# rookiepig/CrossScalePatchMatch

Hardware: AMD Instinct MI355X
Metric: Mpix/s disparity (GRD, use_cs=true) (higher is better)
Workload: dtype f64; 1 GPU; C3: 1242x375 max_dis=128 GRD scale_num=5 reg_lambda=0.3 wnd=35 iters=3 (BASELINE.json configs[2] when C3); cc_name=GRD, schedule=raster, sweep_cells=as cost_source, raster_sweep=persistent, rb_rounds=1, sweep_workgroups_per_cu=2, sweep_workgroup_waves=levels - 1 (coarsest level folded, CSPM_OPT_SWEEP_FOLD), early_exit=True, pairs_per_gpu=22, distinct_pairs_per_gpu=22, pairs_in_flight_per_gpu=2, use_pp=False, parallelism=1 rank(s), one per GPU, 2 independent pair stream(s) each, dispatch=every rank generates its own pairs (no collective in the timed region)

## Files before the change

### crossscalepatchmatch_amd/csrc/cspm_chain.h

```cpp
#pragma once
#include <type_traits>
#include "cspm_tap.h"

#pragma clang fp contract(off)

namespace cspm {

struct ChainScratch {
  double part[2][kMaxPasses * kWave];
};
struct ChainPlane { double a, b, c; };

struct ChainLevel {
  int W, H, n, Dm1;
  int ox0, oy0;
  int r_lo, nrows;
  int passes, nsteps;
  int Wp, pad;
  bool has_valid;
  double maxc;
  const char *px, *opx;
  const char *gx, *ogx;
  int dirE;
  double sgn;
  const double *vol;
  const char *vol2;
  size_t slab;
  uint32_t Ip;
};

template <int SRC>
__device__ __forceinline__ ChainLevel make_chain_level(const Cost &cd, int s, int view, int cx, int cy) {
  const Level &L = cd.lv[s];
  constexpr int E = elem_size<SRC>();
  ChainLevel A;
  A.W = L.W; A.H = L.H; A.n = cd.n; A.Dm1 = L.D - 1;
  A.ox0 = cx - cd.half; A.oy0 = cy - cd.half;
  A.r_lo = max(0, -A.oy0);
  const int r_hi = min(cd.n - 1, L.H - 1 - A.oy0);
  A.nrows = r_hi - A.r_lo + 1;
  A.passes = (A.nrows + kChainRows - 1) / kChainRows;
  A.nsteps = (cd.n + kRowMod - 1) / kRowMod;
  A.Wp = L.Wp; A.pad = L.pad;
  A.has_valid = L.D >= 2;
  A.maxc = cd.max_cost[view * CSPM_MAX_LEVELS + s];
  A.vol2 = nullptr;
  A.gx = A.ogx = nullptr;
  if (SRC == kSrcCenGrd) { A.gx = reinterpret_cast<const char *>(L.grd[view]); A.ogx = reinterpret_cast<const char *>(L.grd[1 - view]); }
  if (SRC == kSrcVol2) {
    A.px = reinterpret_cast<const char *>(L.pix[view]); A.opx = A.px;
    A.Ip = L.pix[view][cy * L.Wp + L.pad + cx];
    A.vol2 = reinterpret_cast<const char *>(L.vol2[view]);
    A.Dm1 = max(L.D - 1, 1);
  } else if (census_elem<SRC>()) {
    A.px = reinterpret_cast<const char *>(L.pc[view]); A.opx = reinterpret_cast<const char *>(L.pc[1 - view]);
    A.Ip = L.pc[view][cy * L.Wp + L.pad + cx].pix;
  } else if (SRC == kSrcGrd8) {
    A.px = reinterpret_cast<const char *>(L.px8[view]); A.opx = reinterpret_cast<const char *>(L.px8[1 - view]);
    A.Ip = pix8_colour(L.px8[view][cy * L.Wp + L.pad + cx].hi);
  } else {
    A.px = reinterpret_cast<const char *>(L.px[view]); A.opx = reinterpret_cast<const char *>(L.px[1 - view]);
    A.Ip = L.px[view][cy * L.Wp + L.pad + cx].pix;
  }
  A.Ip = (uint32_t)__builtin_amdgcn_readfirstlane((int)A.Ip);
  A.sgn = view == 0 ? -1.0 : 1.0;
  A.dirE = view == 0 ? -E : E;
  A.vol = L.vol[view];
  A.slab = (size_t)L.W * (size_t)L.H;
  return A;
}

#ifdef CSPM_SWEEP_TRACE
constexpr int kTraceSlots = 16;
__shared__ long long *s_tr;
#define EVAL_STAMP(slot) do { if (wave == 0 && lane == 0 && s_tr) s_tr[slot] = wall_clock64(); } while (0)
#else
#define EVAL_STAMP(slot) do { } while (0)
#endif

__device__ __forceinline__ double wave_uniform(double v) {
  return __hiloint2double(__builtin_amdgcn_readfirstlane(__double2hiint(v)), __builtin_amdgcn_readfirstlane(__double2loint(v)));
}

__device__ __forceinline__ void grd8_cell_pair(const double *lut_a, uint32_t Iq, double XP, const uint4 &pr, bool left, double &c0, double &c1) {
  const double clo = grd8_cell(lut_a, Iq, XP, pix8_colour(pr.y), pix8_x(pr.x, pr.y));
  const double chi = grd8_cell(lut_a, Iq, XP, pix8_colour(pr.w), pix8_x(pr.z, pr.w));
  c0 = left ? chi : clo;
  c1 = left ? clo : chi;
}

template <int SRC, bool ALLV>
__device__ __forceinline__ double chain_tap_value(const Cost &cd, const ChainLevel &A, const Luts &lut, const uint4 &P, double XP, double Pg,
                                                  int of, int qx, int qy, bool ok, double q_disp) {
  constexpr int E = SRC == kSrcVol2 ? 4 : elem_size<SRC>();
  if constexpr (SRC == kSrcImg) {
    const ImgSplit g = split_img(q_disp, A.sgn * q_disp, (double)qx, A.Dm1, A.has_valid);
    const int fxc = min(max(g.fx, -A.pad), A.W + A.pad - 2);
    const int oo = (qy * A.Wp + A.pad + fxc) * E;
    const uint4 o0 = ld_elem<SRC>(A.opx, oo), o1 = ld_elem<SRC>(A.opx, oo + E);
    const double cell = img_cell(pix_of<SRC>(P), g_of(P), pix_of<SRC>(o0), g_of(o0), pix_of<SRC>(o1), g_of(o1), g.fw);
    return g.valid ? cell : A.maxc;
  } else {
    const DispSplit d = ALLV ? split_disp_valid(q_disp) : split_disp(q_disp, A.Dm1, A.has_valid);
    double c0, c1;
    if constexpr (SRC == kSrcVol2) {
      const int cx = ok ? qx : A.ox0 + cd.half;
      const unsigned idx = __umul24((unsigned)d.f, (unsigned)A.slab) + (unsigned)(qy * A.W + cx);
      const double2 cc = *reinterpret_cast<const double2 *>(A.vol2 + (size_t)(idx << 4));
      c0 = cc.x;
      c1 = cc.y;
    } else if constexpr (SRC == kSrcVolume) {
      const int cx = ok ? qx : A.ox0 + cd.half;
      const double *v = A.vol + (size_t)d.f * A.slab + (size_t)qy * A.W + cx;
      c0 = v[0];
      c1 = v[A.slab];
    } else if constexpr (SRC == kSrcGrd8) {
      const bool left = A.dirE < 0;
      const uint4 pr = ld_pix8_pair(A.opx, of + __mul24(A.dirE, d.f) + (left ? -E : 0));
      grd8_cell_pair(lut.a, P.z, XP, pr, left, c0, c1);
    } else if constexpr (SRC == kSrcCenGrd) {
      const int oo = of + __mul24(A.dirE, d.f);
      const uint4 o0 = ld_elem<SRC>(A.opx, oo), o1 = ld_elem<SRC>(A.opx, oo + A.dirE);
      const double g0 = ld_grad(A.ogx, oo >> 1), g1 = ld_grad(A.ogx, (oo + A.dirE) >> 1);
      c0 = cengrd_cell(lut.a, P, Pg, o0, g0);
      c1 = cengrd_cell(lut.a, P, Pg, o1, g1);
    } else {
      const int oo = of + __mul24(A.dirE, d.f);
      cell_pair_of<SRC>(lut.a, P, ld_elem<SRC>(A.opx, oo), ld_elem<SRC>(A.opx, oo + A.dirE), c0, c1);
    }
    return ALLV ? lerp_cells(d.fr, c0, c1) : tap_value(d, c0, c1, A.maxc);
  }
}

template <int SRC, int NC, bool PIPE = false>
__device__ __forceinline__ void chain_passes(const Cost &cd, const ChainLevel &A, const Luts &lut, const ChainPlane (&pl)[NC], int lane,
                                             int pass_first, int pass_step, double *const (&part)[NC]) {
  constexpr int E = SRC == kSrcVol2 ? 4 : elem_size<SRC>();
  const int lutzero = kLutZero;
  const int lr = lane / kRowMod, j = lane - lr * kRowMod;
  if constexpr (PIPE && (SRC == kSrcGrd || SRC == kSrcCen || SRC == kSrcGrd8)) {
    struct PassCtx {
      bool chain_ok;
      int ob;
      double ty[NC];
    };
    struct Fetched {
      uint4 P;
      uint4 o0[NC], o1[NC];
      DispSplit d[NC];
      bool ok;
    };
    const double jd = (double)j;
    const int qx0 = A.ox0 + j;
    auto make_ctx = [&](int p) {
      PassCtx c;
      const int r = p * kChainRows + lr;
      c.chain_ok = (lr < kChainRows) & (r < A.nrows);
      const int row = A.oy0 + A.r_lo + (c.chain_ok ? r : 0);
      c.ob = (row * A.Wp + A.pad + qx0) * E;
#pragma unroll
      for (int k = 0; k < NC; ++k) c.ty[k] = pl[k].b * (double)row + pl[k].c;
      return c;
    };
    auto fetch = [&](const PassCtx &c, int st, Fetched &F) {
      const double xg = (double)(A.ox0 + kRowMod * st);
      const int dx = j + kRowMod * st;
      F.ok = c.chain_ok & (dx < A.n) & ((unsigned)(qx0 + kRowMod * st) < (unsigned)A.W);
      if constexpr (SRC == kSrcGrd8) {
        const uint2 e = ld_pix8(A.px, c.ob + st * (kRowMod * E));
        F.P = uint4{e.x, e.y, 0u, 0u};
      } else {
        F.P = ld_elem<SRC>(A.px, c.ob + st * (kRowMod * E));
      }
#pragma unroll
      for (int k = 0; k < NC; ++k) {
        const double q_disp = tap_disp(pl[k].a, jd, group_disp(pl[k].a, xg, c.ty[k]));
        F.d[k] = split_disp(q_disp, A.Dm1, A.has_valid);
        if constexpr (SRC == kSrcGrd8) {
          F.o0[k] = ld_pix8_pair(A.opx, c.ob + st * (kRowMod * E) + __mul24(A.dirE, F.d[k].f) + (A.dirE < 0 ? -E : 0));
        } else {
          const int of = c.ob + st * (kRowMod * E) + __mul24(A.dirE, F.d[k].f);
          F.o0[k] = ld_elem<SRC>(A.opx, of);
          F.o1[k] = ld_elem<SRC>(A.opx, of + A.dirE);
        }
      }
    };
    auto consume = [&](const Fetched &F, double (&acc)[NC]) {
      uint32_t Iq;
      double XP = 0.0;
      if constexpr (SRC == kSrcGrd8) { Iq = pix8_colour(F.P.y); XP = pix8_x(F.P.x, F.P.y); }
      else Iq = pix_of<SRC>(F.P);
      const int sad0 = (int)__builtin_amdgcn_sad_u8(A.Ip, Iq, 0u);
      const int sad = F.ok ? sad0 : lutzero;
      const double wgt = lut.w[sad];
#pragma unroll
      for (int k = 0; k < NC; ++k) {
        double c0, c1;
        if constexpr (SRC == kSrcGrd8) grd8_cell_pair(lut.a, Iq, XP, F.o0[k], A.dirE < 0, c0, c1);
        else cell_pair_of<SRC>(lut.a, F.P, F.o0[k], F.o1[k], c0, c1);
        acc[k] = __builtin_fma(wgt, tap_value(F.d[k], c0, c1, A.maxc), acc[k]);
      }
    };
    auto copy_fetched = [&](Fetched &d, const Fetched &f) {
      d.P = f.P;
      d.ok = f.ok;
#pragma unroll
      for (int k = 0; k < NC; ++k) { d.o0[k] = f.o0[k]; d.o1[k] = f.o1[k]; d.d[k].valid = f.d[k].valid; d.d[k].f = f.d[k].f; d.d[k].fr = f.d[k].fr; }
    };
    auto copy_ctx = [&](PassCtx &d, const PassCtx &c) {
      d.chain_ok = c.chain_ok;
      d.ob = c.ob;
#pragma unroll
      for (int k = 0; k < NC; ++k) d.ty[k] = c.ty[k];
    };
    if (pass_first >= A.passes) return;
    PassCtx cur = make_ctx(pass_first);
    Fetched F0, F1;
    fetch(cur, 0, F0);
    const int nsteps = A.nsteps;
    for (int p = pass_first; p < A.passes; p += pass_step) {
      const bool has_next = p + pass_step < A.passes;
      PassCtx nxt;
      if (has_next) nxt = make_ctx(p + pass_step);
      else copy_ctx(nxt, cur);
      double acc[NC];
#pragma unroll
      for (int k = 0; k < NC; ++k) acc[k] = 0.0;
      int st = 0;
      for (; st + 1 < nsteps; st += 2) {
        fetch(cur, st + 1, F1);
        __builtin_amdgcn_sched_barrier(0);
        consume(F0, acc);
        const bool in2 = st + 2 < nsteps;
        PassCtx cb;
        cb.chain_ok = in2 ? cur.chain_ok : nxt.chain_ok;
        cb.ob = in2 ? cur.ob : nxt.ob;
#pragma unroll
        for (int k = 0; k < NC; ++k) cb.ty[k] = in2 ? cur.ty[k] : nxt.ty[k];
        fetch(cb, in2 ? st + 2 : 0, F0);
        __builtin_amdgcn_sched_barrier(0);
        consume(F1, acc);
      }
      if (st < nsteps) {
        fetch(nxt, 0, F1);
        __builtin_amdgcn_sched_barrier(0);
        consume(F0, acc);
        copy_fetched(F0, F1);
      }
#pragma unroll
      for (int k = 0; k < NC; ++k) part[k][p * kWave + lane] = acc[k];
      copy_ctx(cur, nxt);
    }
    return;
  }
  bool allv = (SRC == kSrcGrd || census_elem<SRC>() || SRC == kSrcGrd8 || SRC == kSrcVolume || SRC == kSrcVol2) && A.has_valid;
  if (allv) {
    const double x0 = (double)A.ox0, x1 = (double)(A.ox0 + kRowMod * A.nsteps - 1);
    const double y0 = (double)(A.oy0 + A.r_lo), y1 = (double)(A.oy0 + A.r_lo + A.nrows - 1);
    const double lo = 1.0 + 0x1p-20, hi = (double)(A.Dm1 + 1) - 0x1p-20;
#pragma unroll
    for (int c = 0; c < NC; ++c) {
      const double t0 = pl[c].b * y0 + pl[c].c, t1 = pl[c].b * y1 + pl[c].c;
      const double q00 = __builtin_fma(pl[c].a, x0, t0), q01 = __builtin_fma(pl[c].a, x1, t0);
      const double q10 = __builtin_fma(pl[c].a, x0, t1), q11 = __builtin_fma(pl[c].a, x1, t1);
      const double qmin = __builtin_fmin(__builtin_fmin(q00, q01), __builtin_fmin(q10, q11));
      const double qmax = __builtin_fmax(__builtin_fmax(q00, q01), __builtin_fmax(q10, q11));
      allv = allv & (qmin >= lo) & (qmax <= hi);
    }
    allv = __builtin_amdgcn_ballot_w64(!allv) == 0ull;
  }
  auto run_passes = [&](auto allv_tag) {
  constexpr bool ALLV = decltype(allv_tag)::value;
  for (int p = pass_first; p < A.passes; p += pass_step) {
    double acc[NC];
#pragma unroll
    for (int c = 0; c < NC; ++c) acc[c] = 0.0;
    const int r = p * kChainRows + lr;
    const bool chain_ok = (lr < kChainRows) & (r < A.nrows);
    const int dy = A.r_lo + (chain_ok ? r : 0);
    const int qx0 = A.ox0 + j;
    const int ob = ((A.oy0 + dy) * A.Wp + A.pad + qx0) * E;
    double ty[NC];
#pragma unroll
    for (int c = 0; c < NC; ++c) ty[c] = pl[c].b * (double)(A.oy0 + dy) + pl[c].c;
    const double jd = (double)j;
    for (int st = 0; st < A.nsteps; ++st) {
      const double xg = (double)(A.ox0 + kRowMod * st);
      const int dx = j + kRowMod * st;
      const bool ok = chain_ok & (dx < A.n) & ((unsigned)(qx0 + kRowMod * st) < (unsigned)A.W);
      uint4 P;
      double XP = 0.0;
      if constexpr (SRC == kSrcVol2) P = uint4{0u, 0u, *reinterpret_cast<const uint32_t *>(A.px + (size_t)(unsigned)(ob + st * (kRowMod * E))), 0u};
      else if constexpr (SRC == kSrcGrd8) {
        const uint2 e = ld_pix8(A.px, ob + st * (kRowMod * E));
        P = uint4{0u, 0u, pix8_colour(e.y), 0u};
        XP = pix8_x(e.x, e.y);
      } else P = ld_elem<SRC>(A.px, ob + st * (kRowMod * E));
      [[maybe_unused]] double Pg = 0.0;
      if constexpr (SRC == kSrcCenGrd) Pg = ld_grad(A.gx, (ob + st * (kRowMod * E)) >> 1);
      const int sad0 = (int)__builtin_amdgcn_sad_u8(A.Ip, (SRC == kSrcVol2 || SRC == kSrcGrd8) ? P.z : pix_of<SRC>(P), 0u);
      const int sad = ok ? sad0 : lutzero;
      const double wgt = lut.w[sad];
#pragma unroll
      for (int c = 0; c < NC; ++c) {
        const double q_disp = tap_disp(pl[c].a, jd, group_disp(pl[c].a, xg, ty[c]));
        acc[c] = __builtin_fma(wgt, chain_tap_value<SRC, ALLV>(cd, A, lut, P, XP, Pg, ob + st * (kRowMod * E), qx0 + kRowMod * st, A.oy0 + dy, ok, q_disp),
                                acc[c]);
      }
    }
#pragma unroll
    for (int c = 0; c < NC; ++c) part[c][p * kWave + lane] = acc[c];
  }
  };
  if (allv) run_passes(std::true_type{});
  else run_passes(std::false_type{});
}

__device__ __forceinline__ double finish_level(const ChainLevel &A, const double *part, int lane) {
  const int r = lane - A.r_lo;
  const bool in = (r >= 0) & (r < A.nrows);
  const int rc = in ? r : 0;
  const int p = rc / kChainRows, lr = rc - p * kChainRows;
  const double *q = part + p * kWave + lr * kRowMod;
  double R = q[0];
#pragma unroll
  for (int k = 1; k < kRowMod; ++k) R = R + q[k];
  R = in ? R : 0.0;
  return wave_tree_sum(R);
}

template <bool CS, int SRC>
__device__ __forceinline__ double eval_plane_chain(const Cost &cd, const Luts &lut, ChainScratch &m, int view, int x, int y, double nx,
                                                   double ny, double nz, double pa, double pb, double pc, double thresh,
                                                   bool use_thresh, int lane) {
  double cost = 0.0;
  double cur_disp = pa * (double)x + pb * (double)y + pc;
  int cur_x = x, cur_y = y;
  const int levels = CS ? cd.levels : 1;
  for (int s = 0; s < levels; ++s) {
    double a = pa, b = pb, c = pc;
    if (CS) plane_param(nx, ny, nz, (double)cur_x, (double)cur_y, cur_disp, a, b, c);
    const ChainLevel A = make_chain_level<SRC>(cd, s, view, cur_x, cur_y);
    const ChainPlane pl[1] = {{wave_uniform(a), wave_uniform(b), wave_uniform(c)}};
    double *const parts[1] = {m.part[0]};
    wave_lds_fence();
    chain_passes<SRC, 1, true>(cd, A, lut, pl, lane, 0, 1, parts);
    wave_lds_fence();
    const double sc = finish_level(A, m.part[0], lane);
    if (CS) cost += sc * cd.lv[s].wgt;
    else cost = sc;
    if (use_thresh && cost >= thresh) return __builtin_inf();
    cur_y /= 2;
    cur_x /= 2;
    cur_disp /= 2.0;
  }
  return cost;
}

template <bool CS, int SRC>
__global__ __launch_bounds__(kEvalBlock) void k_cost_batch(Cost cd, int view, int n, const int *__restrict__ xy,
                                                           const double *__restrict__ np, double *__restrict__ out) {
  __shared__ LutMem s_lut;
  __shared__ ChainScratch s_m[kEvalBlock / kWave];
  const Luts lut = load_luts(cd, s_lut);
  const int wave = __builtin_amdgcn_readfirstlane((int)(threadIdx.x >> 6));
  const long long e = xcd_block() * (kEvalBlock / kWave) + wave;
  if (e >= n) return;
  const int lane = threadIdx.x & 63;
  const int x = xy[2 * e], y = xy[2 * e + 1];
  const double *p = np + 6 * e;
  const double c = eval_plane_chain<CS, SRC>(cd, lut, s_m[wave], view, x, y, p[0], p[1], p[2], p[3], p[4], p[5], kDoubleMax, false, lane);
  if (lane == 0) out[e] = c;
}

template <bool CS, int SRC>
__global__ __launch_bounds__(kEvalBlock) void k_spatial_rb(Cost cd, Pm pm, int colour, int inc, int nb) {
  __shared__ LutMem s_lut;
  __shared__ ChainScratch s_m[kEvalBlock / kWave];
  const Luts lut = load_luts(cd, s_lut);
  const int halfW = (pm.W + 1) / 2;
  const long long per_view = (long long)halfW * pm.H;
  const int wave = __builtin_amdgcn_readfirstlane((int)(threadIdx.x >> 6));
  const long long e = xcd_block() * (kEvalBlock / kWave) + wave;
  if (e >= 2 * per_view) return;
  const int lane = threadIdx.x & 63;
  const int v = (int)(e / per_view);
  const long long r = e - (long long)v * per_view;
  const int y = (int)(r / halfW);
  const int x = 2 * (int)(r - (long long)y * halfW) + ((y + colour) & 1);
  if (x >= pm.W) return;
  const Field &f = pm.f[v];
  const long long i = (long long)y * pm.W + x;
  Cand best{};
  double best_cost = f.cost[i];
  bool changed = false;
  const bool use_thresh = pm.use_thresh != 0 && *cd.early_ok != 0;
  const int nxs[4] = {x - inc, x, x + inc, x}, nys[4] = {y, y - inc, y, y + inc};
  for (int k = 0; k < nb; ++k) {
    if (nxs[k] < 0 || nxs[k] >= pm.W || nys[k] < 0 || nys[k] >= pm.H) continue;
    const long long j = (long long)nys[k] * pm.W + nxs[k];
    const Cand cand{f.nx[j], f.ny[j], f.nz[j], f.a[j], f.b[j], f.c[j]};
    const double cost = eval_plane_chain<CS, SRC>(cd, lut, s_m[wave], v, x, y, cand.nx, cand.ny, cand.nz, cand.a, cand.b, cand.c, best_cost,
                                                    use_thresh, lane);
    if (cost < best_cost) { best_cost = cost; best = cand; changed = true; }
  }
  if (changed && lane == 0) store_plane(f, i, best.nx, best.ny, best.nz, best.a, best.b, best.c, best_cost);
}

constexpr int kSweepMinWaves = 4;
constexpr int kSweepPollSleep = 1;
constexpr int kSweepPrio = 3;
constexpr int kSweepMaxWaves = CSPM_MAX_LEVELS > kMaxPasses ? CSPM_MAX_LEVELS : kMaxPasses;

struct SweepShared {
  LutMem &lut;
  double (*lvl)[CSPM_MAX_LEVELS];
  ChainScratch *m;
};
__host__ __device__ inline size_t sweep_shared_bytes(int waves) {
  return sizeof(LutMem) + 2 * CSPM_MAX_LEVELS * sizeof(double) + (size_t)(waves < 1 ? 1 : waves) * sizeof(ChainScratch);
}
__device__ __forceinline__ SweepShared sweep_shared(unsigned char *smem) {
  return SweepShared{*reinterpret_cast<LutMem *>(smem), reinterpret_cast<double (*)[CSPM_MAX_LEVELS]>(smem + sizeof(LutMem)),
                     reinterpret_cast<ChainScratch *>(smem + sizeof(LutMem) + 2 * CSPM_MAX_LEVELS * sizeof(double))};
}

template <bool CS, int SRC>
__device__ __forceinline__ ChainLevel sweep_level_setup(const Cost &cd, int v, int x, int y, int wave) {
  if (CS) {
    int cur_x = x, cur_y = y;
    for (int s = 0; s < wave; ++s) { cur_y /= 2; cur_x /= 2; }
    return make_chain_level<SRC>(cd, wave < cd.levels ? wave : 0, v, cur_x, cur_y);
  }
  return make_chain_level<SRC>(cd, 0, v, x, y);
}

template <bool CS, int SRC>
__device__ __forceinline__ void eval_pixel_pair(const Cost &cd, const Luts &lut, const SweepShared &sh, int v, int x, int y, const Cand &c0,
                                                const Cand &c1, bool both, int wave, int lane, double &cost0, double &cost1, const ChainLevel &A) {
  if (CS) {
    const int level = wave;
    double d0 = c0.a * (double)x + c0.b * (double)y + c0.c, d1 = c1.a * (double)x + c1.b * (double)y + c1.c;
    int cur_x = x, cur_y = y;
    for (int s = 0; s < level; ++s) { cur_y /= 2; cur_x /= 2; d0 /= 2.0; d1 /= 2.0; }
    double *part0 = sh.m[level].part[0], *part1 = sh.m[level].part[1];
    if (level < cd.levels) {
      const double wgt = cd.lv[level].wgt;
      ChainPlane pl[2];
      plane_param(c0.nx, c0.ny, c0.nz, (double)cur_x, (double)cur_y, d0, pl[0].a, pl[0].b, pl[0].c);
      pl[0].a = wave_uniform(pl[0].a); pl[0].b = wave_uniform(pl[0].b); pl[0].c = wave_uniform(pl[0].c);
      if (both) {
        plane_param(c1.nx, c1.ny, c1.nz, (double)cur_x, (double)cur_y, d1, pl[1].a, pl[1].b, pl[1].c);
        pl[1].a = wave_uniform(pl[1].a); pl[1].b = wave_uniform(pl[1].b); pl[1].c = wave_uniform(pl[1].c);
        EVAL_STAMP(4);
        double *const parts[2] = {part0, part1};
        chain_passes<SRC, 2>(cd, A, lut, pl, lane, 0, 1, parts);
        EVAL_STAMP(5);
        wave_lds_fence();
        const double s0 = finish_level(A, part0, lane) * wgt;
        const double s1 = finish_level(A, part1, lane) * wgt;
        if (lane == 0) { sh.lvl[0][level] = s0; sh.lvl[1][level] = s1; }
      } else {
        const ChainPlane p1[1] = {pl[0]};
        double *const parts[1] = {part0};
        chain_passes<SRC, 1>(cd, A, lut, p1, lane, 0, 1, parts);
        wave_lds_fence();
        const double s0 = finish_level(A, part0, lane) * wgt;
        if (lane == 0) { sh.lvl[0][level] = s0; sh.lvl[1][level] = s0; }
      }
    }
    const int nw = (int)(blockDim.x >> 6);
    if (cd.levels == nw + 1) {
      const int last = cd.levels - 1;
      double *fold0 = sh.m[nw].part[0], *fold1 = sh.m[nw].part[1];
      ChainLevel B = A;
      if (wave >= 1) {
        double e0 = c0.a * (double)x + c0.b * (double)y + c0.c, e1 = c1.a * (double)x + c1.b * (double)y + c1.c;
        int lx = x, ly = y;
        for (int s = 0; s < last; ++s) { ly /= 2; lx /= 2; e0 /= 2.0; e1 /= 2.0; }
        B = make_chain_level<SRC>(cd, last, v, lx, ly);
        ChainPlane pl[2];
        plane_param(c0.nx, c0.ny, c0.nz, (double)lx, (double)ly, e0, pl[0].a, pl[0].b, pl[0].c);
        pl[0].a = wave_uniform(pl[0].a); pl[0].b = wave_uniform(pl[0].b); pl[0].c = wave_uniform(pl[0].c);
        if (both) {
          plane_param(c1.nx, c1.ny, c1.nz, (double)lx, (double)ly, e1, pl[1].a, pl[1].b, pl[1].c);
          pl[1].a = wave_uniform(pl[1].a); pl[1].b = wave_uniform(pl[1].b); pl[1].c = wave_uniform(pl[1].c);
          double *const parts[2] = {fold0, fold1};
          chain_passes<SRC, 2>(cd, B, lut, pl, lane, wave - 1, nw - 1, parts);
        } else {
          const ChainPlane p1[1] = {pl[0]};
          double *const parts[1] = {fold0};
          chain_passes<SRC, 1>(cd, B, lut, p1, lane, wave - 1, nw - 1, parts);
        }
      }
      __syncthreads();
      if (wave == 1) {
        const double s0 = finish_level(B, fold0, lane) * cd.lv[last].wgt;
        if (lane == 0) { sh.lvl[0][last] = s0; if (!both) sh.lvl[1][last] = s0; }
      } else if (wave == 2 && both) {
        const double s1 = finish_level(B, fold1, lane) * cd.lv[last].wgt;
        if (lane == 0) sh.lvl[1][last] = s1;
      }
    }
    __syncthreads();
    cost0 = cost1 = 0.0;
    if (wave == 0) {
      for (int s = 0; s < cd.levels; ++s) {
        cost0 += sh.lvl[0][s];
        cost1 += sh.lvl[1][s];
      }
    }
  } else {
    const int nw = (int)(blockDim.x >> 6);
    const ChainPlane pl[2] = {{wave_uniform(c0.a), wave_uniform(c0.b), wave_uniform(c0.c)}, {wave_uniform(c1.a), wave_uniform(c1.b), wave_uniform(c1.c)}};
    double *const parts[2] = {sh.m[0].part[0], sh.m[0].part[1]};
    if (both) {
      chain_passes<SRC, 2>(cd, A, lut, pl, lane, wave, nw, parts);
    } else {
      const ChainPlane p1[1] = {pl[0]};
      double *const parts1[1] = {parts[0]};
      chain_passes<SRC, 1>(cd, A, lut, p1, lane, wave, nw, parts1);
    }
    __syncthreads();
    cost0 = cost1 = 0.0;
    if (wave == 0) {
      cost0 = finish_level(A, parts[0], lane);
      cost1 = both ? finish_level(A, parts[1], lane) : cost0;
    }
  }
}


__device__ __forceinline__ void sweep_candidates(const double (*pl)[6], const double *own_k, long long own_stride, bool have0, bool have1, bool trust, Cand &c0, Cand &c1,
                                                 bool &eval0, bool &eval1) {
  const int p0 = have0 ? 0 : 1, p1 = have1 ? 1 : 0;
  c0 = Cand{pl[p0][0], pl[p0][1], pl[p0][2], pl[p0][3], pl[p0][4], pl[p0][5]};
  c1 = Cand{pl[p1][0], pl[p1][1], pl[p1][2], pl[p1][3], pl[p1][4], pl[p1][5]};
  const Cand own{own_k[0], own_k[own_stride], own_k[2 * own_stride], own_k[3 * own_stride], own_k[4 * own_stride], own_k[5 * own_stride]};
  const bool same01 = c0.nx == c1.nx && c0.ny == c1.ny && c0.nz == c1.nz && c0.a == c1.a && c0.b == c1.b && c0.c == c1.c;
  const bool own0 = same_plane(c0, own, trust);
  const bool own1 = same_plane(c1, own, trust);
  eval0 = have0 && !own0;
  eval1 = have1 && !own1 && !(have0 && same01);
}
__device__ __forceinline__ int sweep_accept(bool eval0, double cost0, bool eval1, double cost1, double &best_cost) {
  int pick = -1;
  if (eval0 && cost0 < best_cost) { best_cost = cost0; pick = 0; }
  if (eval1 && cost1 < best_cost) { best_cost = cost1; pick = 1; }
  return pick;
}

template <bool CS, int SRC>
__global__ __launch_bounds__(kSweepMaxWaves *kWave) void k_spatial_diag(Cost cd, Pm pm, int k, int inc) {
  extern __shared__ __attribute__((aligned(16))) unsigned char smem[];
  const SweepShared sh = sweep_shared(smem);
  const Luts lut = load_luts(cd, sh.lut);
  const int ys_lo = max(0, k - (pm.W - 1)), ys_hi = min(pm.H - 1, k);
  const int cnt = ys_hi - ys_lo + 1;
  const int b = (int)blockIdx.x;
  const int v = b / cnt;
  const int ys = ys_lo + (b - v * cnt), xs = k - ys;
  const int x = inc > 0 ? xs : pm.W - 1 - xs, y = inc > 0 ? ys : pm.H - 1 - ys;
  const Field &f = pm.f[v];
  const long long i = (long long)y * pm.W + x;
  const int wave = __builtin_amdgcn_readfirstlane((int)(threadIdx.x >> 6));
  const int lane = threadIdx.x & 63;
  const bool have0 = xs > 0, have1 = ys > 0;
  if (!have0 && !have1) return;
  const long long jx = i - inc, jy = i - (long long)inc * pm.W;
  const long long j0 = have0 ? jx : jy, j1 = have1 ? jy : jx;
  const Cand c0{f.nx[j0], f.ny[j0], f.nz[j0], f.a[j0], f.b[j0], f.c[j0]};
  const Cand c1{f.nx[j1], f.ny[j1], f.nz[j1], f.a[j1], f.b[j1], f.c[j1]};
  const bool same01 = same_plane(c0, c1);
  double cost0, cost1;
  const ChainLevel A = sweep_level_setup<CS, SRC>(cd, v, x, y, wave);
  eval_pixel_pair<CS, SRC>(cd, lut, sh, v, x, y, c0, c1, have0 && have1 && !same01, wave, lane, cost0, cost1, A);
  if (threadIdx.x == 0) {
    double best_cost = f.cost[i];
    const int pick = sweep_accept(have0, cost0, have1, cost1, best_cost);
    if (pick >= 0) store_plane(f, i, pick == 0 ? c0 : c1, best_cost);
  }
}

constexpr int kGranPerPixel = 12;
constexpr int kSweepMaxBands = 8;
struct Sweep {
  unsigned int *ctrl;
  unsigned long long *gran[2];
  const unsigned int *start;
  int nbands;
  unsigned int epoch, total;
  long long timeout_ticks;
  long long *trace;
  unsigned int *ready[2];
  unsigned long long *queue;
  unsigned int *qctl;
};
#ifdef CSPM_SWEEP_TRACE
#define SWEEP_STAMP(slot) do { if (threadIdx.x == 0 && sw.trace) sw.trace[((size_t)2 * pm.W * by0 + item) * kTraceSlots + (slot)] = wall_clock64(); } while (0)
#else
#define SWEEP_STAMP(slot) do { } while (0)
#endif

__device__ __forceinline__ bool wait_granules(const unsigned long long *p, bool need, unsigned int epoch, unsigned int *err, long long timeout_ticks,
                                              unsigned long long &g) {
  const long long t0 = wall_clock64();
  g = 0ull;
  for (unsigned spins = 1;; ++spins) {
    if (need) g = __hip_atomic_load(p, __ATOMIC_RELAXED, __HIP_MEMORY_SCOPE_AGENT);
    const bool ready = !need || (unsigned int)(g >> 32) == epoch;
    if (__builtin_amdgcn_ballot_w64(!ready) == 0ull) return true;
    __builtin_amdgcn_s_sleep(kSweepPollSleep);
    if ((spins & 255u) == 0u) {
      if (__hip_atomic_load(err, __ATOMIC_RELAXED, __HIP_MEMORY_SCOPE_AGENT) != 0u) return false;
      if (wall_clock64() - t0 > timeout_ticks) {
        __hip_atomic_store(err, 1u, __ATOMIC_RELAXED, __HIP_MEMORY_SCOPE_AGENT);
        return false;
      }
    }
  }
}

template <bool CS, int SRC>
__global__ __launch_bounds__(kSweepMaxWaves *kWave, kSweepMinWaves) void k_spatial_sweep(Cost cd, Pm pm, Sweep sw, int inc) {
  extern __shared__ __attribute__((aligned(16))) unsigned char smem[];
  const SweepShared sh = sweep_shared(smem);
  __shared__ double s_plane[2][2][6];
  __shared__ double s_own[2][8];
  __shared__ unsigned int s_item[2];
  __shared__ int s_ok;
  const Luts lut = load_luts(cd, sh.lut);
  __builtin_amdgcn_s_setprio(kSweepPrio);
  const int wave = __builtin_amdgcn_readfirstlane((int)(threadIdx.x >> 6));
  const int lane = threadIdx.x & 63;
  const int ndiag = pm.W + pm.H - 1;
  const int band = (int)(blockIdx.x % (unsigned)sw.nbands);
  const int by0 = (int)((long long)band * pm.H / sw.nbands), by1 = (int)((long long)(band + 1) * pm.H / sw.nbands);
  const unsigned int *bstart = sw.start + (size_t)band * (size_t)(ndiag + 1);
  const unsigned int btotal = bstart[ndiag];
  unsigned int *claim = &sw.ctrl[2 + band];
  int k = by0;
  if (threadIdx.x == 0) {
    if (__hip_atomic_load(&sw.ctrl[1], __ATOMIC_RELAXED, __HIP_MEMORY_SCOPE_AGENT) != 0u) s_item[0] = btotal;
    else s_item[0] = __hip_atomic_fetch_add(claim, 1u, __ATOMIC_RELAXED, __HIP_MEMORY_SCOPE_AGENT);
    s_ok = 1;
  }
  __syncthreads();
  for (unsigned int par = 0;; par ^= 1u) {
    const unsigned int item = s_item[par];
    if (item >= btotal) return;
    unsigned int next_item = 0;
    if (threadIdx.x == 0) next_item = __hip_atomic_fetch_add(claim, 1u, __ATOMIC_RELAXED, __HIP_MEMORY_SCOPE_AGENT);
    SWEEP_STAMP(0);
#ifdef CSPM_SWEEP_TRACE
    if (threadIdx.x == 0) { s_tr = sw.trace ? sw.trace + ((size_t)2 * pm.W * by0 + item) * kTraceSlots : nullptr; if (s_tr) { s_tr[4] = 0; s_tr[5] = 0; for (int k = 8; k < kTraceSlots; ++k) s_tr[k] = 0; } }
    {
      __shared__ unsigned int s_hwid[kSweepMaxWaves];
      unsigned int hwid, xcc;
      asm volatile("s_getreg_b32 %0, hwreg(HW_REG_HW_ID)" : "=s"(hwid));
      asm volatile("s_getreg_b32 %0, hwreg(HW_REG_XCC_ID)" : "=s"(xcc));
      if (lane == 0) s_hwid[wave] = hwid;
      __syncthreads();
      if (threadIdx.x == 0 && sw.trace) {
        long long packed = 0;
        for (int k = 0; k < (int)(blockDim.x >> 6) && k < 5; ++k) packed |= (long long)(s_hwid[k] & 0xFFFu) << (12 * k);
        sw.trace[((size_t)2 * pm.W * by0 + item) * kTraceSlots + 14] = packed;
        sw.trace[((size_t)2 * pm.W * by0 + item) * kTraceSlots + 15] = (long long)(((s_hwid[0] >> 13) & 7u) | ((xcc & 0xFu) << 4));
      }
    }
#endif
    while (k + 1 < ndiag && item >= bstart[k + 1]) ++k;
    const int ys_lo = max(by0, k - (pm.W - 1)), ys_hi = min(by1 - 1, k);
    const int cnt = ys_hi - ys_lo + 1;
    const int r = (int)(item - bstart[k]);
    const int v = r / cnt;
    const int ys = ys_lo + (r - v * cnt), xs = k - ys;
    const int x = inc > 0 ? xs : pm.W - 1 - xs, y = inc > 0 ? ys : pm.H - 1 - ys;
    const Field &f = pm.f[v];
    const long long i = (long long)y * pm.W + x;
    const long long jx = i - inc, jy = i - (long long)inc * pm.W;
    const bool have0 = xs > 0, have1 = ys > 0;
    SWEEP_STAMP(1);
    const ChainLevel A = sweep_level_setup<CS, SRC>(cd, v, x, y, wave);
    if (wave == 0) {
      const long long comp = f.ny - f.nx;
      double mine = 0.0;
      if (lane < 6) mine = f.nx[lane * comp + i];
      else if (lane == 6) mine = f.cost[i];
      const int pred = lane >= kGranPerPixel ? 1 : 0, part = lane - pred * kGranPerPixel;
      const bool need = lane < 2 * kGranPerPixel && (pred == 0 ? have0 : have1);
      unsigned long long g;
      const bool ok = wait_granules(sw.gran[v] + (pred == 0 ? jx : jy) * kGranPerPixel + (need ? part : 0), need, sw.epoch, &sw.ctrl[1], sw.timeout_ticks, g);
      if (lane < 2 * kGranPerPixel) reinterpret_cast<uint32_t *>(&s_plane[par][0][0])[lane] = (uint32_t)g;
      if (lane < 7) s_own[par][lane] = mine;
      if (lane == 0) {
        if (!ok) s_ok = 0;
        s_item[par ^ 1u] = next_item;
      }
    }
    __syncthreads();
    if (!s_ok) return;
    SWEEP_STAMP(2);
    double cost0 = 0.0, cost1 = 0.0;
    bool eval0 = false, eval1 = false;
    const double(*pl)[6] = s_plane[par];
    const double *mine = s_own[par];
    if (have0 || have1) {
      Cand c0, c1;
      sweep_candidates(pl, mine, 1, have0, have1, pm.trust_cost != 0, c0, c1, eval0, eval1);
      SWEEP_STAMP(3);
      if (eval0 && eval1) {
        eval_pixel_pair<CS, SRC>(cd, lut, sh, v, x, y, c0, c1, true, wave, lane, cost0, cost1, A);
      } else if (eval0) {
        eval_pixel_pair<CS, SRC>(cd, lut, sh, v, x, y, c0, c0, false, wave, lane, cost0, cost1, A);
      } else if (eval1) {
        eval_pixel_pair<CS, SRC>(cd, lut, sh, v, x, y, c1, c1, false, wave, lane, cost1, cost0, A);
      }
    }
    if (wave == 0) {
      double best_cost = mine[6];
      const int pick = sweep_accept(eval0, cost0, eval1, cost1, best_cost);
      SWEEP_STAMP(6);
      if (lane < kGranPerPixel) {
        const int k = lane >> 1;
        const double val = pick >= 0 ? pl[pick][k] : mine[k];
        const unsigned int half = (lane & 1) ? (unsigned int)__double2hiint(val) : (unsigned int)__double2loint(val);
        __hip_atomic_store(sw.gran[v] + (size_t)i * kGranPerPixel + lane, ((unsigned long long)sw.epoch << 32) | half, __ATOMIC_RELAXED,
                           __HIP_MEMORY_SCOPE_AGENT);
      }
      if (pick >= 0) {
        const long long comp = f.ny - f.nx;
        if (lane < 6) f.nx[lane * comp + i] = pl[pick][lane];
        if (lane == 6) f.cost[i] = best_cost;
      }
      SWEEP_STAMP(7);
    }
  }
}

__device__ __forceinline__ void flow_push(const Sweep &sw, unsigned int id) {
  const unsigned int slot = __hip_atomic_fetch_add(&sw.qctl[1], 1u, __ATOMIC_RELAXED, __HIP_MEMORY_SCOPE_AGENT);
  __hip_atomic_store(sw.queue + slot, ((unsigned long long)sw.epoch << 32) | id, __ATOMIC_RELAXED, __HIP_MEMORY_SCOPE_AGENT);
}
__device__ __forceinline__ int flow_pop(const Sweep &sw) {
  if (__hip_atomic_load(&sw.ctrl[1], __ATOMIC_RELAXED, __HIP_MEMORY_SCOPE_AGENT) != 0u) return -1;
  const unsigned int slot = __hip_atomic_fetch_add(&sw.qctl[0], 1u, __ATOMIC_RELAXED, __HIP_MEMORY_SCOPE_AGENT);
  const long long t0 = wall_clock64();
  for (unsigned spins = 1;; ++spins) {
    const unsigned long long e = __hip_atomic_load(sw.queue + slot, __ATOMIC_RELAXED, __HIP_MEMORY_SCOPE_AGENT);
    if ((unsigned int)(e >> 32) == sw.epoch) return (int)(unsigned int)e;
    __builtin_amdgcn_s_sleep(2);
    if ((spins & 15u) == 0u) {
      if (__hip_atomic_load(&sw.qctl[2], __ATOMIC_RELAXED, __HIP_MEMORY_SCOPE_AGENT) >= 2u) return -1;
      if (__hip_atomic_load(&sw.ctrl[1], __ATOMIC_RELAXED, __HIP_MEMORY_SCOPE_AGENT) != 0u) return -1;
      if (wall_clock64() - t0 > sw.timeout_ticks * 4) {
        __hip_atomic_store(&sw.ctrl[1], 1u, __ATOMIC_RELAXED, __HIP_MEMORY_SCOPE_AGENT);
        return -1;
      }
    }
  }
}
#ifdef CSPM_SWEEP_TRACE
#define FLOW_STAMP(slot) do { if (threadIdx.x == 0 && sw.trace) sw.trace[(size_t)item * kTraceSlots + (slot)] = wall_clock64(); } while (0)
#else
#define FLOW_STAMP(slot) do { } while (0)
#endif

template <bool CS, int SRC>
__global__ __launch_bounds__(kSweepMaxWaves *kWave, kSweepMinWaves) void k_spatial_flow(Cost cd, Pm pm, Sweep sw, int inc) {
  extern __shared__ __attribute__((aligned(16))) unsigned char smem[];
  const SweepShared sh = sweep_shared(smem);
  __shared__ double s_plane[2][6];
  __shared__ int s_item, s_from, s_ok;
  const Luts lut = load_luts(cd, sh.lut);
  __builtin_amdgcn_s_setprio(kSweepPrio);
  const int wave = __builtin_amdgcn_readfirstlane((int)(threadIdx.x >> 6));
  const int lane = threadIdx.x & 63;
  const unsigned int npix = (unsigned int)pm.W * (unsigned int)pm.H;
  if (blockIdx.x == 0 && threadIdx.x == 0) {
    const unsigned int origin = inc > 0 ? 0u : npix - 1u;
    flow_push(sw, origin);
    flow_push(sw, npix + origin);
  }
  int next = -1, carry = -1;
  for (;;) {
    if (threadIdx.x == 0) {
      int it = next, from = carry;
      if (it < 0) { it = flow_pop(sw); from = -1; }
      s_item = it;
      s_from = from;
      s_ok = 1;
    }
    __syncthreads();
    const int item = s_item;
    if (item < 0) return;
    const int from = s_from;
    FLOW_STAMP(0);
#ifdef CSPM_SWEEP_TRACE
    if (threadIdx.x == 0) { s_tr = sw.trace ? sw.trace + (size_t)item * kTraceSlots : nullptr; if (s_tr) { s_tr[4] = 0; s_tr[5] = 0; for (int k = 8; k < kTraceSlots; ++k) s_tr[k] = 0; s_tr[15] = from; } }
#endif
    const int v = (unsigned int)item >= npix ? 1 : 0;
    const int pix = item - v * (int)npix;
    const int y = pix / pm.W, x = pix - y * pm.W;
    const int xs = inc > 0 ? x : pm.W - 1 - x, ys = inc > 0 ? y : pm.H - 1 - y;
    const Field &f = pm.f[v];
    const long long i = pix;
    const long long jx = i - inc, jy = i - (long long)inc * pm.W;
    const bool have0 = xs > 0, have1 = ys > 0;
    FLOW_STAMP(1);
    unsigned long long g = 0ull;
    const int pred = lane >= kGranPerPixel ? 1 : 0, part = lane - pred * kGranPerPixel;
    const bool need = wave == 0 && lane < 2 * kGranPerPixel && (pred == 0 ? have0 : have1) && pred != from;
    const unsigned long long *gp = sw.gran[v] + (pred == 0 ? jx : jy) * kGranPerPixel + (need ? part : 0);
    if (need) g = __hip_atomic_load(gp, __ATOMIC_RELAXED, __HIP_MEMORY_SCOPE_AGENT);
    const ChainLevel A = sweep_level_setup<CS, SRC>(cd, v, x, y, wave);
    if (wave == 0) {
      bool ok = true;
      if (__builtin_amdgcn_ballot_w64(need && (unsigned int)(g >> 32) != sw.epoch) != 0ull)
        ok = wait_granules(gp, need, sw.epoch, &sw.ctrl[1], sw.timeout_ticks, g);
      if (need) reinterpret_cast<uint32_t *>(&s_plane[0][0])[lane] = (uint32_t)g;
      if (lane == 0 && !ok) s_ok = 0;
    }
    __syncthreads();
    if (!s_ok) return;
    FLOW_STAMP(2);
    double cost0 = 0.0, cost1 = 0.0;
    bool eval0 = false, eval1 = false;
    if (have0 || have1) {
      Cand c0, c1;
      sweep_candidates(s_plane, f.nx + i, f.ny - f.nx, have0, have1, pm.trust_cost != 0, c0, c1, eval0, eval1);
      FLOW_STAMP(3);
      if (eval0 && eval1) {
        eval_pixel_pair<CS, SRC>(cd, lut, sh, v, x, y, c0, c1, true, wave, lane, cost0, cost1, A);
      } else if (eval0) {
        eval_pixel_pair<CS, SRC>(cd, lut, sh, v, x, y, c0, c0, false, wave, lane, cost0, cost1, A);
      } else if (eval1) {
        eval_pixel_pair<CS, SRC>(cd, lut, sh, v, x, y, c1, c1, false, wave, lane, cost1, cost0, A);
      } else {
        __syncthreads();
      }
    } else {
      FLOW_STAMP(3);
      __syncthreads();
    }
    if (wave == 0) {
      double best_cost = f.cost[i];
      const int pick = sweep_accept(eval0, cost0, eval1, cost1, best_cost);
      FLOW_STAMP(6);
      const long long comp = f.ny - f.nx;
      double fin = 0.0;
      if (lane < kGranPerPixel) {
        const int k = lane >> 1;
        fin = pick >= 0 ? s_plane[pick][k] : f.nx[k * comp + i];
        const unsigned int half = (lane & 1) ? (unsigned int)__double2hiint(fin) : (unsigned int)__double2loint(fin);
        __hip_atomic_store(sw.gran[v] + (size_t)i * kGranPerPixel + lane, ((unsigned long long)sw.epoch << 32) | half, __ATOMIC_RELAXED,
                           __HIP_MEMORY_SCOPE_AGENT);
      }
      if (pick >= 0) {
        if (lane < 6) f.nx[lane * comp + i] = s_plane[pick][lane];
        if (lane == 6) f.cost[i] = best_cost;
      }
      const bool ex = lane == 0 ? xs + 1 < pm.W : (lane == 1 ? ys + 1 < pm.H : false);
      const long long si = lane == 0 ? i + inc : i + (long long)inc * pm.W;
      const unsigned int want = lane == 0 ? (ys > 0 ? 2u : 1u) : (xs > 0 ? 2u : 1u);
      bool rdy = false;
      if (ex) rdy = __hip_atomic_fetch_add(sw.ready[v] + si, 1u, __ATOMIC_RELAXED, __HIP_MEMORY_SCOPE_AGENT) + 1u == want;
      const unsigned long long rb = __builtin_amdgcn_ballot_w64(rdy);
      const bool r0 = (rb & 1ull) != 0ull, r1 = (rb & 2ull) != 0ull;
      const int cont = r0 ? 0 : (r1 ? 1 : -1);
      if (lane == 1 && r0 && r1) flow_push(sw, (unsigned int)(v * (int)npix) + (unsigned int)si);
      if (lane == 0) {
        next = cont < 0 ? -1 : v * (int)npix + (int)(cont == 0 ? i + inc : i + (long long)inc * pm.W);
        carry = cont;
        if (xs + 1 == pm.W && ys + 1 == pm.H) __hip_atomic_fetch_add(&sw.qctl[2], 1u, __ATOMIC_RELAXED, __HIP_MEMORY_SCOPE_AGENT);
      }
      if (cont >= 0 && lane < kGranPerPixel && (lane & 1) == 0) s_plane[cont][lane >> 1] = fin;
      FLOW_STAMP(7);
    }
    __syncthreads();
  }
}

}
```

Measured before the change: 3.489 Mpix/s.

## Overlap level setup loads, work claim and granule polling in the sweep loop

Splits chain-level setup into an issue phase and a finish phase, so the centre-pixel and max-cost loads for the own level and the folded coarsest level are issued before the barrier, and the readfirstlane and colour decode run after it. The next work item is now claimed by the last wave, which also advances the diagonal index during the claim instead of every wave scanning bstart. Wave 0 does one speculative relaxed load of the predecessor granules and only enters the polling loop when some lane sees a stale epoch. The goal is to hide global-memory latency and claim/atomic latency behind the dependency wait, at the cost of more register pressure and more complex item bookkeeping.

```diff
diff --git a/crossscalepatchmatch_amd/csrc/cspm_chain.h b/crossscalepatchmatch_amd/csrc/cspm_chain.h
--- a/crossscalepatchmatch_amd/csrc/cspm_chain.h
+++ b/crossscalepatchmatch_amd/csrc/cspm_chain.h
@@ -30,7 +30,14 @@
 };
 
 template <int SRC>
-__device__ __forceinline__ ChainLevel make_chain_level(const Cost &cd, int s, int view, int cx, int cy) {
+__device__ __forceinline__ uint32_t centre_colour(uint32_t word) {
+  if (SRC == kSrcGrd8) word = pix8_colour(word);
+  return (uint32_t)__builtin_amdgcn_readfirstlane((int)word);
+}
+template <int SRC>
+__device__ __forceinline__ void finish_chain_level(ChainLevel &A) { A.Ip = centre_colour<SRC>(A.Ip); }
+template <int SRC>
+__device__ __forceinline__ ChainLevel issue_chain_level(const Cost &cd, int s, int view, int cx, int cy) {
   const Level &L = cd.lv[s];
   constexpr int E = elem_size<SRC>();
   ChainLevel A;
@@ -57,25 +64,35 @@
     A.Ip = L.pc[view][cy * L.Wp + L.pad + cx].pix;
   } else if (SRC == kSrcGrd8) {
     A.px = reinterpret_cast<const char *>(L.px8[view]); A.opx = reinterpret_cast<const char *>(L.px8[1 - view]);
-    A.Ip = pix8_colour(L.px8[view][cy * L.Wp + L.pad + cx].hi);
+    A.Ip = L.px8[view][cy * L.Wp + L.pad + cx].hi;
   } else {
     A.px = reinterpret_cast<const char *>(L.px[view]); A.opx = reinterpret_cast<const char *>(L.px[1 - view]);
     A.Ip = L.px[view][cy * L.Wp + L.pad + cx].pix;
   }
-  A.Ip = (uint32_t)__builtin_amdgcn_readfirstlane((int)A.Ip);
   A.sgn = view == 0 ? -1.0 : 1.0;
   A.dirE = view == 0 ? -E : E;
   A.vol = L.vol[view];
   A.slab = (size_t)L.W * (size_t)L.H;
   return A;
 }
+template <int SRC>
+__device__ __forceinline__ ChainLevel make_chain_level(const Cost &cd, int s, int view, int cx, int cy) {
+  ChainLevel A = issue_chain_level<SRC>(cd, s, view, cx, cy);
+  finish_chain_level<SRC>(A);
+  return A;
+}
 
 #ifdef CSPM_SWEEP_TRACE
 constexpr int kTraceSlots = 16;
 __shared__ long long *s_tr;
 #define EVAL_STAMP(slot) do { if (wave == 0 && lane == 0 && s_tr) s_tr[slot] = wall_clock64(); } while (0)
+#define FOLD_STAMP_OWN() do { if (wave == 1 && lane == 0 && s_tr) s_tr[12] = wall_clock64(); } while (0)
+#define FOLD_STAMP_OFFSET(high) do { if (wave == 1 && lane == 0 && s_tr) { const long long d_ = wall_clock64() - s_tr[12]; \
+    if (high) s_tr[13] |= d_ << 32; else s_tr[13] = d_ & 0xFFFFFFFFll; } } while (0)
 #else
 #define EVAL_STAMP(slot) do { } while (0)
+#define FOLD_STAMP_OWN() do { } while (0)
+#define FOLD_STAMP_OFFSET(high) do { } while (0)
 #endif
 
 __device__ __forceinline__ double wave_uniform(double v) {
@@ -426,18 +443,27 @@
 }
 
 template <bool CS, int SRC>
-__device__ __forceinline__ ChainLevel sweep_level_setup(const Cost &cd, int v, int x, int y, int wave) {
+__device__ __forceinline__ ChainLevel sweep_level_issue(const Cost &cd, int v, int x, int y, int wave) {
   if (CS) {
     int cur_x = x, cur_y = y;
     for (int s = 0; s < wave; ++s) { cur_y /= 2; cur_x /= 2; }
-    return make_chain_level<SRC>(cd, wave < cd.levels ? wave : 0, v, cur_x, cur_y);
-  }
-  return make_chain_level<SRC>(cd, 0, v, x, y);
-}
-
+    return issue_chain_level<SRC>(cd, wave < cd.levels ? wave : 0, v, cur_x, cur_y);
+  }
+  return issue_chain_level<SRC>(cd, 0, v, x, y);
+}
 template <bool CS, int SRC>
+__device__ __forceinline__ ChainLevel sweep_level_setup(const Cost &cd, int v, int x, int y, int wave) {
+  ChainLevel A = sweep_level_issue<CS, SRC>(cd, v, x, y, wave);
+  finish_chain_level<SRC>(A);
+  return A;
+}
+
+struct FoldAhead { uint32_t Ip; double maxc; };
+
+template <bool CS, int SRC, bool AHEAD = false>
 __device__ __forceinline__ void eval_pixel_pair(const Cost &cd, const Luts &lut, const SweepShared &sh, int v, int x, int y, const Cand &c0,
-                                                const Cand &c1, bool both, int wave, int lane, double &cost0, double &cost1, const ChainLevel &A) {
+                                                const Cand &c1, bool both, int wave, int lane, double &cost0, double &cost1, const ChainLevel &A,
+                                                const FoldAhead &fa = FoldAhead{0u, 0.0}) {
   if (CS) {
     const int level = wave;
     double d0 = c0.a * (double)x + c0.b * (double)y + c0.c, d1 = c1.a * (double)x + c1.b * (double)y + c1.c;
@@ -474,24 +500,34 @@
       const int last = cd.levels - 1;
       double *fold0 = sh.m[nw].part[0], *fold1 = sh.m[nw].part[1];
       ChainLevel B = A;
+      FOLD_STAMP_OWN();
       if (wave >= 1) {
         double e0 = c0.a * (double)x + c0.b * (double)y + c0.c, e1 = c1.a * (double)x + c1.b * (double)y + c1.c;
         int lx = x, ly = y;
         for (int s = 0; s < last; ++s) { ly /= 2; lx /= 2; e0 /= 2.0; e1 /= 2.0; }
-        B = make_chain_level<SRC>(cd, last, v, lx, ly);
+        if (AHEAD) {
+          B = issue_chain_level<SRC>(cd, last, v, lx, ly);
+          B.Ip = fa.Ip;
+          B.maxc = fa.maxc;
+        } else {
+          B = make_chain_level<SRC>(cd, last, v, lx, ly);
+        }
         ChainPlane pl[2];
         plane_param(c0.nx, c0.ny, c0.nz, (double)lx, (double)ly, e0, pl[0].a, pl[0].b, pl[0].c);
         pl[0].a = wave_uniform(pl[0].a); pl[0].b = wave_uniform(pl[0].b); pl[0].c = wave_uniform(pl[0].c);
         if (both) {
           plane_param(c1.nx, c1.ny, c1.nz, (double)lx, (double)ly, e1, pl[1].a, pl[1].b, pl[1].c);
           pl[1].a = wave_uniform(pl[1].a); pl[1].b = wave_uniform(pl[1].b); pl[1].c = wave_uniform(pl[1].c);
+          FOLD_STAMP_OFFSET(false);
           double *const parts[2] = {fold0, fold1};
           chain_passes<SRC, 2>(cd, B, lut, pl, lane, wave - 1, nw - 1, parts);
         } else {
+          FOLD_STAMP_OFFSET(false);
           const ChainPlane p1[1] = {pl[0]};
           double *const parts[1] = {fold0};
           chain_passes<SRC, 1>(cd, B, lut, p1, lane, wave - 1, nw - 1, parts);
         }
+        FOLD_STAMP_OFFSET(true);
       }
       __syncthreads();
       if (wave == 1) {
@@ -597,8 +633,10 @@
   unsigned int *qctl;
 };
 #ifdef CSPM_SWEEP_TRACE
-#define SWEEP_STAMP(slot) do { if (threadIdx.x == 0 && sw.trace) sw.trace[((size_t)2 * pm.W * by0 + item) * kTraceSlots + (slot)] = wall_clock64(); } while (0)
+#define SWEEP_STAMP_ANY(slot) do { if (sw.trace) sw.trace[((size_t)2 * pm.W * by0 + item) * kTraceSlots + (slot)] = wall_clock64(); } while (0)
+#define SWEEP_STAMP(slot) do { if (threadIdx.x == 0) SWEEP_STAMP_ANY(slot); } while (0)
 #else
+#define SWEEP_STAMP_ANY(slot) do { } while (0)
 #define SWEEP_STAMP(slot) do { } while (0)
 #endif
 
@@ -621,13 +659,30 @@
   }
 }
 
+__device__ __forceinline__ uint4 sweep_claim(unsigned int *claim, const unsigned int *bstart, int ndiag, unsigned int btotal, int k, unsigned int bk) {
+  const unsigned int e1 = bstart[min(k + 1, ndiag)], e2 = bstart[min(k + 2, ndiag)];
+  const unsigned int it = __hip_atomic_fetch_add(claim, 1u, __ATOMIC_RELAXED, __HIP_MEMORY_SCOPE_AGENT);
+  if (it < btotal && k + 1 < ndiag && it >= e1) {
+    ++k; bk = e1;
+    if (k + 1 < ndiag && it >= e2) {
+      ++k; bk = e2;
+      while (k + 1 < ndiag) {
+        const unsigned int e = bstart[k + 1];
+        if (it < e) break;
+        ++k; bk = e;
+      }
+    }
+  }
+  return uint4{it, (unsigned int)k, bk, 0u};
+}
+
 template <bool CS, int SRC>
 __global__ __launch_bounds__(kSweepMaxWaves *kWave, kSweepMinWaves) void k_spatial_sweep(Cost cd, Pm pm, Sweep sw, int inc) {
   extern __shared__ __attribute__((aligned(16))) unsigned char smem[];
   const SweepShared sh = sweep_shared(smem);
   __shared__ double s_plane[2][2][6];
   __shared__ double s_own[2][8];
-  __shared__ unsigned int s_item[2];
+  __shared__ __attribute__((aligned(16))) unsigned int s_item[2][4];
   __shared__ int s_ok;
   const Luts lut = load_luts(cd, sh.lut);
   __builtin_amdgcn_s_setprio(kSweepPrio);
@@ -637,23 +692,27 @@
   const int band = (int)(blockIdx.x % (unsigned)sw.nbands);
   const int by0 = (int)((long long)band * pm.H / sw.nbands), by1 = (int)((long long)(band + 1) * pm.H / sw.nbands);
   const unsigned int *bstart = sw.start + (size_t)band * (size_t)(ndiag + 1);
-  const unsigned int btotal = bstart[ndiag];
+  const unsigned int btotal = (unsigned int)__builtin_amdgcn_readfirstlane((int)bstart[ndiag]);
   unsigned int *claim = &sw.ctrl[2 + band];
-  int k = by0;
-  if (threadIdx.x == 0) {
-    if (__hip_atomic_load(&sw.ctrl[1], __ATOMIC_RELAXED, __HIP_MEMORY_SCOPE_AGENT) != 0u) s_item[0] = btotal;
-    else s_item[0] = __hip_atomic_fetch_add(claim, 1u, __ATOMIC_RELAXED, __HIP_MEMORY_SCOPE_AGENT);
+  const bool claims = wave == (int)(blockDim.x >> 6) - 1;
+  if (claims && lane == 0) {
+    uint4 first{btotal, 0u, 0u, 0u};
+    if (__hip_atomic_load(&sw.ctrl[1], __ATOMIC_RELAXED, __HIP_MEMORY_SCOPE_AGENT) == 0u)
+      first = sweep_claim(claim, bstart, ndiag, btotal, by0, bstart[by0]);
+    *reinterpret_cast<uint4 *>(s_item[0]) = first;
     s_ok = 1;
   }
   __syncthreads();
   for (unsigned int par = 0;; par ^= 1u) {
-    const unsigned int item = s_item[par];
+    const uint4 it = *reinterpret_cast<const uint4 *>(s_item[par]);
+    const unsigned int item = (unsigned int)__builtin_amdgcn_readfirstlane((int)it.x);
     if (item >= btotal) return;
-    unsigned int next_item = 0;
-    if (threadIdx.x == 0) next_item = __hip_atomic_fetch_add(claim, 1u, __ATOMIC_RELAXED, __HIP_MEMORY_SCOPE_AGENT);
+    const int k = __builtin_amdgcn_readfirstlane((int)it.y);
+    const unsigned int bk = (unsigned int)__builtin_amdgcn_readfirstlane((int)it.z);
+    SWEEP_STAMP(8);
     SWEEP_STAMP(0);
 #ifdef CSPM_SWEEP_TRACE
-    if (threadIdx.x == 0) { s_tr = sw.trace ? sw.trace + ((size_t)2 * pm.W * by0 + item) * kTraceSlots : nullptr; if (s_tr) { s_tr[4] = 0; s_tr[5] = 0; for (int k = 8; k < kTraceSlots; ++k) s_tr[k] = 0; } }
+    if (threadIdx.x == 0) { s_tr = sw.trace ? sw.trace + ((size_t)2 * pm.W * by0 + item) * kTraceSlots : nullptr; if (s_tr) { s_tr[4] = 0; s_tr[5] = 0; for (int k = 10; k < kTraceSlots; ++k) s_tr[k] = 0; } }
     {
       __shared__ unsigned int s_hwid[kSweepMaxWaves];
       unsigned int hwid, xcc;
@@ -669,10 +728,9 @@
       }
     }
 #endif
-    while (k + 1 < ndiag && item >= bstart[k + 1]) ++k;
     const int ys_lo = max(by0, k - (pm.W - 1)), ys_hi = min(by1 - 1, k);
     const int cnt = ys_hi - ys_lo + 1;
-    const int r = (int)(item - bstart[k]);
+    const int r = (int)(item - bk);
     const int v = r / cnt;
     const int ys = ys_lo + (r - v * cnt), xs = k - ys;
     const int x = inc > 0 ? xs : pm.W - 1 - xs, y = inc > 0 ? ys : pm.H - 1 - ys;
@@ -681,25 +739,48 @@
     const long long jx = i - inc, jy = i - (long long)inc * pm.W;
     const bool have0 = xs > 0, have1 = ys > 0;
     SWEEP_STAMP(1);
-    const ChainLevel A = sweep_level_setup<CS, SRC>(cd, v, x, y, wave);
+    unsigned long long g = 0ull;
+    const unsigned long long *gp = nullptr;
+    bool need = false;
+    double own_word = 0.0;
     if (wave == 0) {
+      const int pred = lane >= kGranPerPixel ? 1 : 0, part = lane - pred * kGranPerPixel;
+      need = lane < 2 * kGranPerPixel && (pred == 0 ? have0 : have1);
+      gp = (v == 0 ? sw.gran[0] : sw.gran[1]) + (pred == 0 ? jx : jy) * kGranPerPixel + (need ? part : 0);
+      if (need) g = __hip_atomic_load(gp, __ATOMIC_RELAXED, __HIP_MEMORY_SCOPE_AGENT);
+      SWEEP_STAMP(11);
       const long long comp = f.ny - f.nx;
-      double mine = 0.0;
-      if (lane < 6) mine = f.nx[lane * comp + i];
-      else if (lane == 6) mine = f.cost[i];
-      const int pred = lane >= kGranPerPixel ? 1 : 0, part = lane - pred * kGranPerPixel;
-      const bool need = lane < 2 * kGranPerPixel && (pred == 0 ? have0 : have1);
-      unsigned long long g;
-      const bool ok = wait_granules(sw.gran[v] + (pred == 0 ? jx : jy) * kGranPerPixel + (need ? part : 0), need, sw.epoch, &sw.ctrl[1], sw.timeout_ticks, g);
+      if (lane < 6) own_word = f.nx[lane * comp + i];
+      else if (lane == 6) own_word = f.cost[i];
+    }
+    ChainLevel A = sweep_level_issue<CS, SRC>(cd, v, x, y, wave);
+    FoldAhead fa{0u, 0.0};
+    const bool folds = CS && wave >= 1 && cd.levels == (int)(blockDim.x >> 6) + 1;
+    if (folds) {
+      int lx = x, ly = y;
+      for (int s = 0; s < cd.levels - 1; ++s) { ly /= 2; lx /= 2; }
+      const ChainLevel F = issue_chain_level<SRC>(cd, cd.levels - 1, v, lx, ly);
+      fa.Ip = F.Ip;
+      fa.maxc = F.maxc;
+    }
+    if (claims && lane == 0) {
+      *reinterpret_cast<uint4 *>(s_item[par ^ 1u]) = sweep_claim(claim, bstart, ndiag, btotal, k, bk);
+      SWEEP_STAMP_ANY(9);
+    }
+    const bool late = __builtin_amdgcn_ballot_w64(need && (unsigned int)(g >> 32) != sw.epoch) != 0ull;
+    if (wave == 0) {
+      bool ok = true;
+      if (late) ok = wait_granules(gp, need, sw.epoch, &sw.ctrl[1], sw.timeout_ticks, g);
       if (lane < 2 * kGranPerPixel) reinterpret_cast<uint32_t *>(&s_plane[par][0][0])[lane] = (uint32_t)g;
-      if (lane < 7) s_own[par][lane] = mine;
-      if (lane == 0) {
-        if (!ok) s_ok = 0;
-        s_item[par ^ 1u] = next_item;
-      }
+      if (lane < 7) s_own[par][lane] = own_word;
+      if (lane == 0 && !ok) s_ok = 0;
     }
     __syncthreads();
     if (!s_ok) return;
+    finish_chain_level<SRC>(A);
+    fa.Ip = centre_colour<SRC>(fa.Ip);
+    fa.maxc = wave_uniform(fa.maxc);
+    SWEEP_STAMP(10);
     SWEEP_STAMP(2);
     double cost0 = 0.0, cost1 = 0.0;
     bool eval0 = false, eval1 = false;
@@ -710,11 +791,11 @@
       sweep_candidates(pl, mine, 1, have0, have1, pm.trust_cost != 0, c0, c1, eval0, eval1);
       SWEEP_STAMP(3);
       if (eval0 && eval1) {
-        eval_pixel_pair<CS, SRC>(cd, lut, sh, v, x, y, c0, c1, true, wave, lane, cost0, cost1, A);
+        eval_pixel_pair<CS, SRC, true>(cd, lut, sh, v, x, y, c0, c1, true, wave, lane, cost0, cost1, A, fa);
       } else if (eval0) {
-        eval_pixel_pair<CS, SRC>(cd, lut, sh, v, x, y, c0, c0, false, wave, lane, cost0, cost1, A);
+        eval_pixel_pair<CS, SRC, true>(cd, lut, sh, v, x, y, c0, c0, false, wave, lane, cost0, cost1, A, fa);
       } else if (eval1) {
-        eval_pixel_pair<CS, SRC>(cd, lut, sh, v, x, y, c1, c1, false, wave, lane, cost1, cost0, A);
+        eval_pixel_pair<CS, SRC, true>(cd, lut, sh, v, x, y, c1, c1, false, wave, lane, cost1, cost0, A, fa);
       }
     }
     if (wave == 0) {
```

Measured after the change: 3.527 Mpix/s, median of 5. 1.1% higher.
